# TheRealShamsaba/KnightVision

Measured on AMD Instinct MI355X. Metric: MCTS simulations/sec + self-play games/hour, higher is better.
Workload: dtype fp32

## Files before the change

### include/kv.h

```cpp
#ifndef KV_H
#define KV_H

#include <stddef.h>
#include <stdint.h>

#ifdef __cplusplus
extern "C" {
#endif

#define KV_OK 0
#define KV_EINVAL -1
#define KV_ENOMEM -2
#define KV_EHIP -3
#define KV_EOVERFLOW -4

const char* kv_last_error(void);
int kv_version(void);

typedef struct kv_net kv_net;

size_t kv_net_packed_size(void);
int kv_net_create(int device, kv_net** out);
int kv_net_load(kv_net* net, const float* packed, size_t n_floats);
int kv_net_forward(kv_net* net, const float* planes_dev, int B, float* policy_dev, float* value_dev, void* stream);
// ... 183 lines not shown
                       int8_t* states_after, uint8_t* in_check);
int kv_dev_attacks(int device, const int8_t* states, int n, uint64_t* attacked);
int kv_dev_make_move(int device, int8_t* states, const int* index, int n);
int kv_dev_dirichlet(int device, const uint64_t* seeds, int n, double alpha, int k, int draws, double* out,
                     int64_t* attempts, double* tail);
int kv_dev_eval_cache(int device, int entries, const int8_t* boards, const uint16_t* moves, const int* counts,
                      const uint32_t* logits, const uint32_t* values, int n_rows, const int* step_len, int n_steps,
                      int32_t* hit, uint32_t* out_logits, uint32_t* out_values, int64_t* counters);
int kv_host_libm(int op, const double* x, const double* y, int n, double* out);
int kv_dev_py_random(int device, const uint64_t* seeds, int n, int count, double* out);
int kv_dev_wino88i(int device, const double* V, int rows, const double* U, int K, int digits, int seg, double* M,
                   int8_t* v_digits, int* v_exp);
int kv_dev_wino88i32_out(int device, const float* M, int rows, const float* scale, const float* shift,
                         const float* resid, int fused, float* Y, int8_t* v_digits, int* v_exp);
int kv_dev_tower_front(int device, const int8_t* boards, int nb, int rows, const float* wT, const float* scale,
                       const float* shift, int fused, int8_t* v_digits, int* v_exp);
int kv_dev_tower_back(int device, const float* M, int rows, const float* scale, const float* shift,
                      const float* resid, const float* heads, int fused, float* pfeat, float* value);
int kv_dev_wino88r_out(int device, const double* M, int rows, const float* scale, const float* shift,
                       const float* resid, int fused, float* Y, int8_t* v_digits, int* v_exp);
int kv_dev_net_pair(kv_net* a, kv_net* b, int cu_share, int follow);
int kv_dev_i8gemm_bench(int device, int rows, int K, int variant, int iters, float* avg_us, float* M_out);
int kv_dev_gemm_clock(int device, int rows, int digits, double seconds, double* out);
int kv_dev_out_phases(int device, int rows, int resid, int r3, unsigned long long* stamps, float* us);

#define KV_PGN_OUTCOME_NONE (-128)
typedef struct kv_pgn_record {
    char fen[100];
    char san[12];
    int32_t outcome;
    int32_t game;
} kv_pgn_record;
int kv_pgn_extract(const char* text, size_t len, kv_pgn_record* out, size_t cap, size_t* n_out, size_t* consumed,
                   int64_t* n_games);
int kv_fen_codes(const char* fens, size_t stride, int n, int8_t* codes);
int kv_san_move_index(const char* fens, size_t fen_stride, const char* sans, size_t san_stride, int n,
                      int32_t* out);
int kv_chess_perft(const char* fen, int depth, uint64_t* nodes);
int kv_chess_san(const char* fen, const char* san_in, char* san_out, size_t san_cap, char* fen_after, size_t fen_cap);
int kv_chess_fen(const char* fen_in, char* fen_out, size_t cap);

int kv_tr_conv3x3_f16(const void* x_dev, int n, int ci, const void* w_dev, const float* bias_dev, int co,
                      void* y_dev, void* stream);
int kv_tr_conv3x3_add_f16(const void* x_dev, int n, int ci, const void* w_dev, const float* bias_dev, int co,
                          const void* add_dev, void* y_dev, void* stream);
int kv_tr_conv_weights_f16(const float* w_dev, int co, int ci_real, int ci, void* wf_dev, void* wt_dev, void* stream);
// ... 34 lines not shown
```

### knightvision_amd/_lib.py

```python
from __future__ import annotations

import ctypes as C
import os

HERE = os.path.dirname(os.path.abspath(__file__))
LIB_PATH = os.environ.get("KV_LIB_PATH") or os.path.join(HERE, "libkv.so")

_lib = None


class KVError(RuntimeError):
    pass


class Config(C.Structure):
    _fields_ = [("device", C.c_int), ("slots", C.c_int), ("n_games", C.c_int64), ("game_id_base", C.c_int64),
                ("game_id_stride", C.c_int64), ("seed", C.c_uint64), ("seed_mode", C.c_int),
                ("max_moves", C.c_int), ("batch", C.c_int), ("eps", C.c_double), ("alpha", C.c_double),
                ("sims", C.c_int), ("c_puct", C.c_float), ("eval_mode", C.c_int), ("record_cap", C.c_int64),
                ("recycle", C.c_int), ("precision", C.c_int), ("algo", C.c_int), ("tree_edge_cap", C.c_int),
                ("keep_root_visits", C.c_int), ("eval_cache", C.c_int), ("leaves", C.c_int), ("arena", C.c_int), ("sample_plies", C.c_int),
                ("sim_groups", C.c_int), ("reuse_tree", C.c_int)]


# ... 104 lines not shown
        "kv_root_visits_device": ([vp, vp, sz, P(sz), vp], i),
        "kv_root_moves": ([vp, P(C.c_uint16), sz, P(sz)], i),
        "kv_root_moves_device": ([vp, vp, sz, P(sz), vp], i),
        "kv_records_device": ([vp, vp, sz, P(sz), vp], i),
        "kv_sync": ([vp], i),
        "kv_reset_records": ([vp], i),
        "kv_destroy": ([vp], None),
        "kv_search": ([vp, P(C.c_int8), i, P(SearchParams), P(SearchResult)], i),
        "kv_sizeof_search_result": ([], sz),
        "kv_search_advance": ([vp, i, P(C.c_int32), P(C.c_int8)], i),
        "kv_search_continue": ([vp, i, P(SearchParams), P(SearchResult), P(C.c_int32)], i),
        "kv_search_tree_size": ([vp, i, P(C.c_int32), P(C.c_int32)], i),
        "kv_dev_valid_moves": ([i, P(C.c_int8), i, P(C.c_uint16), i, P(i), P(C.c_int8), P(C.c_uint8)], i),
        "kv_dev_make_move": ([i, P(C.c_int8), P(i), i], i),
        "kv_dev_attacks": ([i, P(C.c_int8), i, P(C.c_uint64)], i),
        "kv_dev_dirichlet": ([i, P(C.c_uint64), i, C.c_double, i, i, P(C.c_double), P(i64), P(C.c_double)], i),
        "kv_dev_py_random": ([i, P(C.c_uint64), i, i, P(C.c_double)], i),
        "kv_dev_eval_cache": ([i, i, P(C.c_int8), P(C.c_uint16), P(i), P(C.c_uint32), P(C.c_uint32), i, P(i), i,
                               P(C.c_int32), P(C.c_uint32), P(C.c_uint32), P(i64)], i),
        "kv_host_libm": ([i, P(C.c_double), P(C.c_double), i, P(C.c_double)], i),
        "kv_dev_wino88i": ([i, P(C.c_double), i, P(C.c_double), i, i, i, P(C.c_double), P(C.c_int8), P(i)], i),
        "kv_dev_i8gemm_bench": ([i, i, i, i, i, P(C.c_float), P(C.c_float)], i),
        "kv_dev_gemm_clock": ([i, i, i, C.c_double, P(C.c_double)], i),
        "kv_dev_net_pair": ([vp, vp, i, i], i),
        "kv_dev_out_phases": ([i, i, i, i, P(C.c_uint64), P(C.c_float)], i),
        "kv_dev_wino88i32_out": ([i, P(C.c_float), i, P(C.c_float), P(C.c_float), P(C.c_float), i, P(C.c_float),
                                  P(C.c_int8), P(i)], i),
        "kv_dev_tower_front": ([i, P(C.c_int8), i, i, P(C.c_float), P(C.c_float), P(C.c_float), i, P(C.c_int8),
                                P(i)], i),
        "kv_dev_tower_back": ([i, P(C.c_float), i, P(C.c_float), P(C.c_float), P(C.c_float), P(C.c_float), i,
                               P(C.c_float), P(C.c_float)], i),
        "kv_dev_wino88r_out": ([i, P(C.c_double), i, P(C.c_float), P(C.c_float), P(C.c_float), i, P(C.c_float),
                                P(C.c_int8), P(i)], i),
        "kv_pgn_extract": ([C.c_char_p, sz, P(PgnRecord), sz, P(sz), P(sz), P(i64)], i),
        "kv_fen_codes": ([C.c_char_p, sz, i, P(C.c_int8)], i),
        "kv_san_move_index": ([C.c_char_p, sz, C.c_char_p, sz, i, P(C.c_int32)], i),
        "kv_chess_perft": ([C.c_char_p, i, P(C.c_uint64)], i),
        "kv_chess_san": ([C.c_char_p, C.c_char_p, C.c_char_p, sz, C.c_char_p, sz], i),
        "kv_chess_fen": ([C.c_char_p, C.c_char_p, sz], i),
        "kv_tr_conv3x3_f16": ([vp, i, i, vp, vp, i, vp, vp], i),
        "kv_tr_conv3x3_add_f16": ([vp, i, i, vp, vp, i, vp, vp, vp], i),
        "kv_tr_conv_weights_f16": ([vp, i, i, i, vp, vp, vp], i),
        "kv_tr_wgrad_workspace": ([i, i, i, P(i)], sz),
        "kv_tr_conv3x3_wgrad_f16": ([vp, vp, i, i, i, i, vp, vp, sz, vp], i),
        "kv_tr_bn_workspace": ([i, i], sz),
        "kv_tr_bn_stats_f16": ([vp, i, i, C.c_float, vp, vp, vp, vp, sz, vp], i),
# ... 4 lines not shown
        "kv_tr_head1x1_f16": ([vp, i, vp, vp, vp, vp], i),
        "kv_tr_head1x1_workspace": ([i], sz),
        "kv_tr_head1x1_backward_f16": ([vp, vp, i, vp, vp, vp, vp, vp, sz, vp], i),
        "kv_tr_policy_loss_f16": ([vp, vp, vp, vp, vp, i, vp, vp, vp, vp], i),
        "kv_tr_policy_loss_backward_f16": ([vp, vp, vp, vp, vp, i, vp, vp, vp, vp, vp, vp], i),
    }
    for name, (args, res) in sig.items():
        if not hasattr(L, name):
            continue
        f = getattr(L, name)
        f.argtypes = args
        f.restype = res
    return L


EXPORTED = ["kv_last_error", "kv_version", "kv_net_packed_size", "kv_net_create", "kv_net_load", "kv_net_forward",
            "kv_net_forward_boards", "kv_net_forward_boards_legal", "kv_net_set_timing", "kv_net_last_timing", "kv_net_destroy", "kv_net_set_precision", "kv_net_set_algo",
            "kv_net_calibration", "kv_engine_calibration",
            "kv_create", "kv_sim_groups_for",
            "kv_load_weights", "kv_load_weights_b", "kv_engine_calibration_b", "kv_run", "kv_set_max_moves", "kv_records", "kv_games", "kv_stats_get", "kv_sizeof_config", "kv_sizeof_stats", "kv_root_visits", "kv_root_visits_device", "kv_root_moves", "kv_root_moves_device", "kv_records_device", "kv_sync", "kv_reset_records", "kv_destroy",
            "kv_search", "kv_sizeof_search_result", "kv_search_advance", "kv_search_continue", "kv_search_tree_size",
            "kv_dev_valid_moves", "kv_dev_make_move", "kv_dev_attacks", "kv_dev_dirichlet", "kv_dev_py_random", "kv_host_libm", "kv_dev_eval_cache",
            "kv_dev_wino88i", "kv_dev_wino88i32_out", "kv_dev_wino88r_out", "kv_dev_tower_front", "kv_dev_tower_back", "kv_dev_i8gemm_bench",
            "kv_dev_gemm_clock", "kv_dev_out_phases", "kv_dev_net_pair",
            "kv_pgn_extract", "kv_fen_codes", "kv_san_move_index", "kv_chess_perft", "kv_chess_san", "kv_chess_fen",
            "kv_tr_conv3x3_f16", "kv_tr_conv3x3_add_f16", "kv_tr_conv_weights_f16", "kv_tr_wgrad_workspace", "kv_tr_conv3x3_wgrad_f16",
            "kv_tr_bn_workspace", "kv_tr_bn_stats_f16", "kv_tr_bn_apply_f16", "kv_tr_bn_backward_f16",
            "kv_tr_channel_sum_f16", "kv_tr_planes_to_nhwc", "kv_tr_head1x1_f16", "kv_tr_head1x1_workspace",
            "kv_tr_head1x1_backward_f16", "kv_tr_policy_loss_f16", "kv_tr_policy_loss_backward_f16"]


def lib():
    global _lib
    if _lib is None:
        import torch
        if not os.path.exists(LIB_PATH):
            raise KVError(f"{LIB_PATH} is missing: run `python -c 'import __graft_entry__ as g; g.build()'` "
                          "(the HIP library is required; there is no CPU fallback)")
        L = _declare(C.CDLL(LIB_PATH))
        if hasattr(L, "kv_sizeof_search_result"):
            assert L.kv_sizeof_search_result() == C.sizeof(SearchResult), "kv_search_result: ctypes mirror differs"
        if hasattr(L, "kv_sizeof_config"):
            assert L.kv_sizeof_config() == C.sizeof(Config), "kv_config: ctypes mirror differs"
            assert L.kv_sizeof_stats() == C.sizeof(Stats), "kv_stats: ctypes mirror differs"
        _lib = L
    return _lib

# ... 6 lines not shown
```

### knightvision_amd/csrc/kv_nn.hip

```cpp
#include <hip/hip_runtime.h>
#include <math.h>
#include <stdarg.h>
#include <stdlib.h>
#include <string.h>

#include <algorithm>
#include <chrono>
#include <mutex>
#include <set>
#include <utility>
#include <vector>

#include "kv_common.h"
#include "kv_wino.h"
#include "kv_wino88.h"
#include "kv_wino88d.h"
#include "kv_wino88i.h"
#include "kv_ref64.h"

namespace kv {

static thread_local char g_err[512];

void set_error(const char* fmt, ...) {
// ... 960 lines not shown
    KV_HIP(hipGetLastError());
    return KV_OK;
}

#ifndef KV_I8F32_NB
#define KV_I8F32_NB 3
#endif
template <int K, int TPW, int ND = 4, int LJ = KV_I8F32_LJ, int NB = KV_I8F32_NB>
static int launch_wino88i32_gemm_lagt(const int8_t* V8, const int* ev, const int8_t* U8, const int* eu, float* M,
                                      int rows, int stride, hipStream_t st) {
    using T = kv::Wino88iTile<kv::kI8DigitsF32>;
    constexpr int bytes = NB * T::STAGE;
    auto kern = kv::wino88i32_gemm_lagt_kernel<K, TPW, LJ, false, ND, NB>;
    KV_HIP(lds_opt_in((const void*)kern, bytes));
    const int tiles = kv::W88_XI * (rows / T::WM) * (512 / T::WN);
    KV_REQUIRE(rows % T::WM == 0 && stride % T::WM == 0 && tiles % (8 * TPW) == 0, KV_EINVAL,
               "wino gemm i8 (lagt): rows %d / stride %d vs tile %d", rows, stride, T::WM);
    hipLaunchKernelGGL(kern, dim3(tiles / TPW), dim3(T::THREADS), bytes, st, V8, ev, U8, eu, M, rows, 512, stride,
                       nullptr);
    KV_HIP(hipGetLastError());
    return KV_OK;
}

template <int K, int TPW>
static int launch_wino88i32_gemm_r3k64(const int8_t* V8, const int* ev, const int8_t* U8, const int* eu, float* M,
                                       int rows, int stride, hipStream_t st, int share = 1) {
    constexpr int bytes = 3 * 4 * 128 * 96 + 2 * TPW * 1024;
    auto kern = kv::wino88i32_gemm_r3k64_kernel<K, TPW>;
    if constexpr (K == 512 && TPW == 5) {
        static const int abl = [] {
            const char* e = getenv("KV_R3K64_ABL");
            return e ? atoi(e) : 0;
        }();
        if (abl == 1) kern = kv::wino88i32_gemm_r3k64_kernel<K, TPW, false, 1>;
        if (abl == 2) kern = kv::wino88i32_gemm_r3k64_kernel<K, TPW, false, 2>;
        if (abl == 3) kern = kv::wino88i32_gemm_r3k64_kernel<K, TPW, false, 3>;
        if (abl == 4) kern = kv::wino88i32_gemm_r3k64_kernel<K, TPW, false, 4>;
        if (abl == 7) kern = kv::wino88i32_gemm_r3k64_kernel<K, TPW, false, 7>;
        if (abl == 8) kern = kv::wino88i32_gemm_r3k64_kernel<K, TPW, false, 8>;
    }
    KV_HIP(lds_opt_in((const void*)kern, bytes));
    const int tiles = kv::W88_XI * (rows / 128) * (512 / 128);
    KV_REQUIRE(rows % 128 == 0 && stride % 128 == 0 && tiles % (8 * TPW) == 0, KV_EINVAL,
               "wino gemm i8 (r3k64): rows %d / stride %d vs tile 128", rows, stride);
    int nwg = tiles / TPW;
    const int cus = gemm_cus(share);
    if (r3_one_round() && cus > 0 && cus % 8 == 0 && nwg > cus && nwg % cus == 0) nwg = cus;
    KV_REQUIRE(nwg % 8 == 0 && tiles % (nwg * TPW) == 0, KV_EINVAL, "wino gemm i8 (r3k64): %d tiles, %d workgroups",
               tiles, nwg);
    hipLaunchKernelGGL(kern, dim3(nwg), dim3(512), bytes, st, V8, ev, U8, eu, M, rows, 512, stride, nullptr);
    KV_HIP(hipGetLastError());
    return KV_OK;
}

static int i8f32_tiles_per_wg(int rows, int share = 1) {
    static const bool off = [] {
        const char* e = getenv("KV_I8F32_TPW");
        return e && e[0] == '1';
    }();
    const int cus = gemm_cus(share);
    const int tiles = kv::W88_XI * (rows / 128) * 4;
    if (off || cus <= 0) return 1;
    const int single = (tiles + cus - 1) / cus;
    for (int t = 5; t >= 4; --t) {
        if (tiles % (8 * t)) continue;
        const int wgs = tiles / t;
        if ((wgs + cus - 1) / cus * t <= single) return t;
    }
    return 1;
}
// ... 1021 lines not shown
    } else {
        constexpr int D = kv::kI8DigitsF32;
        rc = K == 256 ? launch_wino88i_slice<256, D>(du.p, 512, 512, kv::W88_XI, u8.p, eu.p, 0)
                      : launch_wino88i_slice<512, D>(du.p, 512, 512, kv::W88_XI, u8.p, eu.p, 0);
        if (!rc)
            rc = K == 256 ? launch_wino88i_slice<256, D>(dv.p, rows, rows, kv::W88_XI, v8.p, ev.p, 0)
                 : seg    ? launch_wino88i_slice<512, D, double, 2>(dv.p, rows, rows, kv::W88_XI, v8.p, ev.p, 0)
                          : launch_wino88i_slice<512, D>(dv.p, rows, rows, kv::W88_XI, v8.p, ev.p, 0);
        if (!rc)
            rc = K == 256 ? i8f32_gemm<256>(v8.p, ev.p, u8.p, eu.p, dmf.p, rows, rows, false, 0)
                          : i8f32_gemm<512>(v8.p, ev.p, u8.p, eu.p, dmf.p, rows, rows, seg != 0, 0);
    }
    if (rc) return rc;
    KV_HIP(hipDeviceSynchronize());
    if (digits == 5 || r8) {
        KV_HIP(hipMemcpy(M, dm.p, nm * sizeof(double), hipMemcpyDeviceToHost));
    } else {
        std::vector<float> mf(nm);
        KV_HIP(hipMemcpy(mf.data(), dmf.p, nm * sizeof(float), hipMemcpyDeviceToHost));
        for (size_t i = 0; i < nm; ++i) M[i] = mf[i];
    }
    if (v_digits) KV_HIP(hipMemcpy(v_digits, v8.p, nv * digits, hipMemcpyDeviceToHost));
    if (v_exp) KV_HIP(hipMemcpy(v_exp, ev.p, (size_t)kv::W88_XI * rows * nseg * sizeof(int), hipMemcpyDeviceToHost));
    return KV_OK;
}

}

template <bool RESID, bool R3>
static void dev_out_rowform(int form, const float* M, int rows, const float* sc, const float* sh, float* y,
                            int8_t* v8, int* ev) {
    const float* rs = RESID ? y : nullptr;
    if (form == 2)
        (void)launch_wino88i32_outp<RESID, true>(M, rows, rows, sc, sh, rs, y, v8, ev, 0, R3);
    else if (form == 0)
        hipLaunchKernelGGL((kv::wino88i32_out_kernel<RESID, true, 512, R3>), dim3(1, rows), dim3(1024), 0, 0, M, rows,
                           sc, sh, rs, y, v8, ev, 0, 0);
    else
        hipLaunchKernelGGL((kv::wino88i32_out2_kernel<RESID, true, R3>), dim3(1, rows), dim3(1024), 0, 0, M, rows, sc,
                           sh, rs, y, v8, ev, 0, 0);
}

extern "C" {

int kv_dev_wino88i32_out(int device, const float* M, int rows, const float* scale, const float* shift,
                         const float* resid, int fused, float* Y, int8_t* v_digits, int* v_exp) {
// ... 317 lines not shown
                return k5 ? launch_wino88i32_gemm<512, 64, 2, 1, 0, true>(v8.p, ev.p, u8.p, eu.p, m.p, rows, rows, true, 0)
                          : launch_wino88i32_gemm<256, 64, 2, 1, 0, true>(v8.p, ev.p, u8.p, eu.p, m.p, rows, rows, true, 0);
            default: KV_REQUIRE(false, KV_EINVAL, "kv_dev_i8gemm_bench: variant %d", variant);
        }
    };
    int rc;
    for (int w = 0; w < 2; ++w)
        if ((rc = run())) return rc;
    kv::DevEvent e0, e1;
    KV_HIP(e0.create());
    KV_HIP(e1.create());
    KV_HIP(hipEventRecord(e0.e, 0));
    for (int it = 0; it < iters; ++it)
        if ((rc = run())) return rc;
    KV_HIP(hipEventRecord(e1.e, 0));
    KV_HIP(hipEventSynchronize(e1.e));
    float ms = 0.f;
    KV_HIP(hipEventElapsedTime(&ms, e0.e, e1.e));
    *avg_us = 1000.f * ms / iters;
    if (M_out) KV_HIP(hipMemcpy(M_out, m.p, nm * sizeof(float), hipMemcpyDeviceToHost));
    return KV_OK;
}

int kv_dev_gemm_clock(int device, int rows, int digits, double seconds, double* out) {
    KV_REQUIRE(rows > 0 && rows % 128 == 0 && rows <= kMaxBoards && (digits == 3 || digits == 4) && seconds > 0 && out,
               KV_EINVAL, "kv_dev_gemm_clock: bad arguments (rows %d: a multiple of 128, at most %d; digits %d: 3 or 4)",
               rows, kMaxBoards, digits);
    const bool r3 = digits == 3;
    KV_HIP(hipSetDevice(device));
    constexpr int K = 512;
    const size_t lv = (size_t)kv::W88_XI * (K / 32) * rows, lu = (size_t)kv::W88_XI * (K / 32) * 512;
    const size_t nm = (size_t)kv::W88_XI * rows * 512;
    kv::DevBuf<int8_t> v8, u8;
    kv::DevBuf<int> ev, eu;
    kv::DevBuf<float> m;
    kv::DevBuf<unsigned long long> stamps;
    KV_HIP(v8.alloc(lv * 128));
    KV_HIP(u8.alloc(lu * 128));
    KV_HIP(ev.alloc((size_t)kv::W88_XI * rows * 2));
    KV_HIP(eu.alloc((size_t)kv::W88_XI * 512));
    KV_HIP(m.alloc(nm));
    hipLaunchKernelGGL(i8_fill_kernel, dim3((unsigned)((lv * 128 + 255) / 256)), dim3(256), 0, 0, v8.p, lv, ev.p,
                       (size_t)kv::W88_XI * rows * 2, 1234u);
    hipLaunchKernelGGL(i8_fill_kernel, dim3((unsigned)((lu * 128 + 255) / 256)), dim3(256), 0, 0, u8.p, lu, eu.p,
                       (size_t)kv::W88_XI * 512, 99u);
    KV_HIP(hipGetLastError());
    int rc;
    for (int w = 0; w < 3; ++w)
        if ((rc = i8f32_gemm<K>(v8.p, ev.p, u8.p, eu.p, m.p, rows, rows, false, 0, r3))) return rc;
    KV_HIP(hipDeviceSynchronize());
    kv::DevEvent e0, e1;
    KV_HIP(e0.create());
    KV_HIP(e1.create());
    int launches = 0;
    const auto t_start = std::chrono::steady_clock::now();
    KV_HIP(hipEventRecord(e0.e, 0));
    while (std::chrono::duration<double>(std::chrono::steady_clock::now() - t_start).count() < seconds) {
        for (int i = 0; i < 50; ++i)
            if ((rc = i8f32_gemm<K>(v8.p, ev.p, u8.p, eu.p, m.p, rows, rows, false, 0, r3))) return rc;
        launches += 50;
        KV_HIP(hipStreamSynchronize(0));
    }
    KV_HIP(hipEventRecord(e1.e, 0));
    KV_HIP(hipEventSynchronize(e1.e));
    float ms = 0.f;
    KV_HIP(hipEventElapsedTime(&ms, e0.e, e1.e));
    using T = kv::Wino88iTile<kv::kI8DigitsF32>;
    const int tpw = i8f32_tiles_per_wg(rows) >= 4 ? i8f32_tiles_per_wg(rows) : 1;
    const int tiles = kv::W88_XI * (rows / T::WM) * (512 / T::WN), nwg = tiles / tpw;
    KV_REQUIRE(tiles % (8 * tpw) == 0, KV_EINVAL, "kv_dev_gemm_clock: %d tiles, %d per workgroup", tiles, tpw);
    KV_HIP(stamps.alloc((size_t)nwg * 4));
    const int bytes = r3 ? 3 * 4 * 128 * 96 + 2 * tpw * 1024 : KV_I8F32_NB * T::STAGE;
    auto kern = r3 ? (tpw == 5   ? kv::wino88i32_gemm_r3k64_kernel<K, 5, true>
                      : tpw == 4 ? kv::wino88i32_gemm_r3k64_kernel<K, 4, true>
                                 : kv::wino88i32_gemm_r3k64_kernel<K, 1, true>)
                   : (tpw == 5   ? kv::wino88i32_gemm_lagt_kernel<K, 5, KV_I8F32_LJ, true, 4, KV_I8F32_NB>
                      : tpw == 4 ? kv::wino88i32_gemm_lagt_kernel<K, 4, KV_I8F32_LJ, true, 4, KV_I8F32_NB>
                                 : kv::wino88i32_gemm_lagt_kernel<K, 1, KV_I8F32_LJ, true, 4, KV_I8F32_NB>);
    KV_HIP(lds_opt_in((const void*)kern, bytes));
    hipLaunchKernelGGL(kern, dim3(nwg), dim3(T::THREADS), bytes, 0, v8.p, ev.p, u8.p, eu.p, m.p, rows, 512, rows,
                       stamps.p);
    KV_HIP(hipGetLastError());
    KV_HIP(hipDeviceSynchronize());
    std::vector<unsigned long long> h((size_t)nwg * 4);
    KV_HIP(hipMemcpy(h.data(), stamps.p, h.size() * sizeof(unsigned long long), hipMemcpyDeviceToHost));
    std::vector<double> mhz;
    mhz.reserve(nwg);
    for (int b = 0; b < nwg; ++b) {
        const double dt = (double)(h[4 * b + 1] - h[4 * b]), dr = (double)(h[4 * b + 3] - h[4 * b + 2]);
        if (dr > 0) mhz.push_back(dt / dr * 100.0);
    }
    KV_REQUIRE(!mhz.empty(), KV_EHIP, "kv_dev_gemm_clock: no stamp pair advanced");
    std::nth_element(mhz.begin(), mhz.begin() + mhz.size() / 2, mhz.end());
    out[0] = mhz[mhz.size() / 2];
    out[1] = 1000.0 * ms / launches;
    out[2] = launches;
    out[3] = tpw;
    return KV_OK;
}

__global__ void out_phase_fill_kernel(float* M, size_t n, float* sc, float* sh) {
    const size_t i = (size_t)blockIdx.x * blockDim.x + threadIdx.x;
    if (i < n) {
        uint32_t z = (uint32_t)(i * 2654435761u) ^ 0x9e3779b9u;
        z ^= z >> 15;
        z *= 0x2c1b3c6du;
        z ^= z >> 12;
        M[i] = ((float)(z & 0xffffff) / 16777216.0f - 0.5f) * 0.6f;
    }
    if (i < 512) {
        sc[i] = 0.5f + (float)(i % 7) * 0.1f;
        sh[i] = -0.01f * (float)(i % 5);
    }
}

int kv_dev_out_phases(int device, int rows, int resid, int r3, unsigned long long* stamps, float* us) {
    KV_REQUIRE(rows > 0 && rows % 128 == 0 && rows <= kMaxBoards && stamps && us, KV_EINVAL,
               "kv_dev_out_phases: bad arguments (rows %d)", rows);
    KV_HIP(hipSetDevice(device));
    const size_t nm = (size_t)kv::W88_XI * rows * 512, ny = (size_t)rows * 64 * 512;
    kv::DevBuf<float> dm, dsc, dsh, dy;
// ... 183 lines not shown
```

### knightvision_amd/csrc/kv_wino88i.h

```cpp
#pragma once
#include <hip/hip_runtime.h>

#include "kv_common.h"
#include "kv_wino88.h"
#include "kv_wino88d.h"

namespace kv {

constexpr int kI8Digits = 5;
constexpr int kI8DigitsF32 = 4;

typedef int i8x16_t __attribute__((ext_vector_type(4)));
typedef int i32x16_t __attribute__((ext_vector_type(16)));

__device__ inline int i8_row_exponent(unsigned m) {
    if (!m) return 0;
    return (int)(m >> 20) - 1022 + ((m & 0xFE000u) == 0xFE000u ? 1 : 0);
}

__device__ inline int i8_row_exponent_f32(unsigned m) {
    if (!m) return 0;
    return (int)(m >> 23) - 126 + ((m & 0x7F0000u) == 0x7F0000u ? 1 : 0);
}

// ... 788 lines not shown
    }
}
#ifndef KV_R3_M_NT
#define KV_R3_M_NT 1
#endif
template <int K, int TPW, bool STAMP = false, int ABL = 0>
__global__ __launch_bounds__(512) void wino88i32_gemm_r3k64_kernel(const int8_t* __restrict__ V8,
                                                                   const int* __restrict__ ev,
                                                                   const int8_t* __restrict__ U8,
                                                                   const int* __restrict__ eu, float* __restrict__ M,
                                                                   int rows, int cout, int stride,
                                                                   unsigned long long* __restrict__ stamps) {
    unsigned long long t0 = 0, r0 = 0;
    if constexpr (STAMP) {
        t0 = __builtin_amdgcn_s_memtime();
        r0 = __builtin_amdgcn_s_memrealtime();
    }
    constexpr int ND = 3, NB = 3, PD = NB - 1, GL = 6;
    constexpr int NT = 2, WM = 128, WN = 128, WC = 2;
    constexpr int NK = K / 32, NU = NK / 2, NSG = TPW * NU;
    constexpr int PLANE = 128 * 96, STAGE = 4 * PLANE;
    static_assert(NK % 2 == 0 && NU > PD && 8 * GL * 1024 == STAGE, "64-k stages, 6 pieces per wave");
    constexpr double kStep = 0.00390625;

    extern __shared__ __attribute__((aligned(16))) i8x16_t lds_i8k64[];
    char* const L0 = (char*)lds_i8k64;

    const int tid = threadIdx.x;
    const int lane = tid & 63, wave = tid >> 6;
    const int wm = wave / WC, wn = wave % WC;
    const int CT = cout / WN, RT = rows / WM;
    const int nwg = (int)gridDim.x, nv = kv::W88_XI * RT * CT, ng = nv / (nwg * TPW), NST = ng * NSG;
    auto coords = [&](int T, int& xi, int& nb, int& rb) {
        const int vb = (int)blockIdx.x + T * nwg;
        const int idx = (vb & 7) * (nv >> 3) + (vb >> 3);
        xi = idx / (CT * RT);
        nb = (idx % CT) * WN;
        rb = ((idx / CT) % RT) * WM;
    };
    int xis[TPW], nbs[TPW], rbs[TPW];

    const int wu = __builtin_amdgcn_readfirstlane(wave);
    const int op = wu >> 2, chunk = (wu >> 1) & 1, pp0 = 6 * (wu & 1);
    const size_t sstep = (op ? (size_t)cout : (size_t)stride) * 96;
    auto tile_base = [&](int xi, int nb, int rb) {
        return (op ? U8 + (((size_t)xi * NK) * cout + (size_t)nb) * 96 : V8 + (((size_t)xi * NK) * stride + (size_t)rb) * 96) +
// ... 7 lines not shown
        goff[g] = (unsigned)(row * 96 + 16 * (slot ^ ((row >> 4) & 1)));
    }
    const int ldst = (op * 2 + chunk) * PLANE + pp0 * 1024;
    auto issue1 = [&](int g, int s, int sg) {
        if constexpr ((ABL & 1) != 0)
            if (sg >= PD) return;
        const int j = s / NU, ku = s - j * NU;
        const int8_t* base = gb[0];
#pragma unroll
        for (int jj = 1; jj <= TPW; ++jj) base = j == jj ? gb[jj] : base;
        const int8_t* const sb = base + (size_t)(2 * ku) * sstep;
#if KV_COPY_SADDR
        const void* src = (const void*)(sb + goff[g]);
#else
        const void* src = (const void*)(sb + (size_t)(int)goff[g]);
#endif
        __builtin_amdgcn_global_load_lds(src,
                                         (__attribute__((address_space(3))) void*)(L0 + (sg % NB) * STAGE + ldst +
                                                                                   g * 1024),
                                         16, 0, 0);
    };

    const int lr = lane & 31, lh = lane >> 5;
    const int arow = wm * 32 + lr;
    int aoff[2][ND], boff[2][NT][ND];
#pragma unroll
    for (int h = 0; h < 2; ++h)
#pragma unroll
        for (int d = 0; d < ND; ++d) {
            aoff[h][d] = h * PLANE + arow * 96 + 16 * ((2 * d + lh) ^ ((arow >> 4) & 1));
#pragma unroll
            for (int nt = 0; nt < NT; ++nt) {
                const int brow = wn * NT * 32 + nt * 32 + lr;
                boff[h][nt][d] = (2 + h) * PLANE + brow * 96 + 16 * ((2 * d + lh) ^ ((brow >> 4) & 1));
            }
        }

    constexpr int NEX = (TPW * 256 + 511) / 512;
    int* const exl = (int*)(L0 + NB * STAGE);
    for (int gi = 0; gi < ng; ++gi) {
#pragma unroll
    for (int j = 0; j < TPW; ++j) {
        coords(gi * TPW + j, xis[j], nbs[j], rbs[j]);
        gb[j] = tile_base(xis[j], nbs[j], rbs[j]);
    }
    {
// ... 15 lines not shown
    if (gi == 0) {
#pragma unroll
        for (int p = 0; p < PD; ++p)
#pragma unroll
            for (int g = 0; g < GL; ++g) issue1(g, p, p);
    }
#pragma unroll
    for (int j = 0; j < TPW; ++j) {
        i32x16_t acc[ND][NT];
#pragma unroll
        for (int l = 0; l < ND; ++l)
#pragma unroll
            for (int nt = 0; nt < NT; ++nt) acc[l][nt] = i32x16_t{};
        i8x16_t pa[2] = {}, pb[2][NT] = {};
        auto h2 = [&]() {
#pragma unroll
            for (int jb = 1; jb < ND; ++jb)
#pragma unroll
                for (int i = 0; i + jb < ND; ++i)
#pragma unroll
                    for (int nt = 0; nt < NT; ++nt)
                        acc[i + jb][nt] = r3mfma<ABL>(pa[i], pb[jb - 1][nt], acc[i + jb][nt]);
        };
        for (int ku = 0; ku < NU; ++ku) {
            const int s = j * NU + ku, sg = gi * NSG + s;
            const int m = NST - 1 - sg < PD - 1 ? NST - 1 - sg : PD - 1;
            if ((gi > 0 || j > 0) && ku < PD) {
                if (m == 0) vm_lgkm_wait<32>();
                else vm_lgkm_wait<GL + 32>();
            } else {
                if (m == 0) vm_lgkm_wait<0>();
                else vm_lgkm_wait<GL>();
            }
            __builtin_amdgcn_s_barrier();
            asm volatile("" ::: "memory");
            const char* buf = L0 + (sg % NB) * STAGE;
            i8x16_t a0[ND], b0[ND][NT], a1[ND], b1[ND][NT];
#pragma unroll
            for (int d = 0; d < ND; ++d) a0[d] = *(const i8x16_t*)(buf + aoff[0][d]);
#pragma unroll
            for (int nt = 0; nt < NT; ++nt) b0[0][nt] = *(const i8x16_t*)(buf + boff[0][nt][0]);
            __builtin_amdgcn_sched_barrier(0);
            if (ku > 0) h2();
            if (sg + PD < NST) {
                issue1(0, s + PD, sg + PD);
                issue1(1, s + PD, sg + PD);
                issue1(2, s + PD, sg + PD);
            }
#pragma unroll
            for (int jb = 0; jb < ND; ++jb) {
                if (jb + 1 < ND) {
#pragma unroll
                    for (int nt = 0; nt < NT; ++nt) b0[jb + 1][nt] = *(const i8x16_t*)(buf + boff[0][nt][jb + 1]);
                } else {
#pragma unroll
                    for (int d = 0; d < ND; ++d) a1[d] = *(const i8x16_t*)(buf + aoff[1][d]);
#pragma unroll
                    for (int nt = 0; nt < NT; ++nt) b1[0][nt] = *(const i8x16_t*)(buf + boff[1][nt][0]);
                }
                __builtin_amdgcn_sched_barrier(0);
#pragma unroll
                for (int i = 0; i + jb < ND; ++i)
#pragma unroll
                    for (int nt = 0; nt < NT; ++nt)
                        acc[i + jb][nt] = r3mfma<ABL>(a0[i], b0[jb][nt], acc[i + jb][nt]);
                if (jb == 0 && sg + PD < NST) {
                    issue1(3, s + PD, sg + PD);
                    issue1(4, s + PD, sg + PD);
                    issue1(5, s + PD, sg + PD);
                }
            }
#pragma unroll
            for (int nt = 0; nt < NT; ++nt) {
                b1[1][nt] = *(const i8x16_t*)(buf + boff[1][nt][1]);
                b1[2][nt] = *(const i8x16_t*)(buf + boff[1][nt][2]);
            }
            __builtin_amdgcn_sched_barrier(0);
#pragma unroll
            for (int i = 0; i < ND; ++i)
#pragma unroll
                for (int nt = 0; nt < NT; ++nt)
                    acc[i][nt] = r3mfma<ABL>(a1[i], b1[0][nt], acc[i][nt]);
            pa[0] = a1[0];
            pa[1] = a1[1];
#pragma unroll
            for (int nt = 0; nt < NT; ++nt) {
                pb[0][nt] = b1[1][nt];
                pb[1][nt] = b1[2][nt];
            }
            if (j == 0 && ku == 1) {
#pragma unroll
                for (int q = 0; q < NEX; ++q)
                    if (tid + q * 512 < TPW * 256) exg[tid + q * 512] = exv[q];
            }
        }
        h2();
        const int xi = xis[j], n_base = nbs[j], r_base = rbs[j];
        const int* evx = exg + j * 256 + wm * 32;
#pragma unroll
        for (int nt = 0; nt < NT; ++nt) {
            const int col = n_base + wn * NT * 32 + nt * 32 + lr;
            const int ec = (ABL & 8) ? -14 : exg[j * 256 + 128 + wn * NT * 32 + nt * 32 + lr] - 14;
#pragma unroll
            for (int r = 0; r < 16; ++r) {
                const int row = (r & 3) + 8 * (r >> 2) + 4 * lh;
                double mm = (double)acc[ND - 1][nt][r];
#pragma unroll
                for (int l = ND - 2; l >= 0; --l) mm = __builtin_fma(mm, kStep, (double)acc[l][nt][r]);
                const float o = (float)ldexp(mm, ((ABL & 8) ? 0 : evx[row]) + ec);
                if constexpr ((ABL & 4) != 0)
                    asm volatile("" ::"v"(o));
                else if constexpr (KV_R3_M_NT)
                    __builtin_nontemporal_store(o, &M[((size_t)xi * stride + r_base + wm * 32 + row) * cout + col]);
                else
                    M[((size_t)xi * stride + r_base + wm * 32 + row) * cout + col] = o;
            }
        }
    }
    }
    if constexpr (STAMP) {
        const unsigned long long t1 = __builtin_amdgcn_s_memtime(), r1 = __builtin_amdgcn_s_memrealtime();
        if (threadIdx.x < 4) {
            const unsigned long long v = threadIdx.x == 0 ? t0 : threadIdx.x == 1 ? t1 : threadIdx.x == 2 ? r0 : r1;
            stamps[(size_t)blockIdx.x * 4 + threadIdx.x] = v;
        }
    }
}

template <int K, int LJ = 3, int S = 5, int RB = 7, bool RL = false>
__global__ __launch_bounds__(512) void wino88i_gemm_lag5_kernel(const int8_t* __restrict__ V8,
                                                                const int* __restrict__ ev,
                                                                const int8_t* __restrict__ U8,
                                                                const int* __restrict__ eu, double* __restrict__ M,
                                                                int rows, int cout, int stride) {
    constexpr int LEV = 5, NBUF = 3;
    using T = Wino88iTile<S>;
    constexpr int NT = T::NT, WM = T::WM, WN = T::WN, GL = T::GL;
    constexpr int NK = K / 32;
    constexpr int NA = S < LEV - LJ ? S : LEV - LJ;
// ... 1062 lines not shown
```

Before: 329,000.

## Overlap r3k64 GEMM epilogue stores with final MFMA stage in multi-tile workgroups

For workgroups that handle several tiles, the last k-stage is reordered so all MFMAs for the first column tile finish first. Its epilogue (digit recombination, ldexp and stores to M) is then interleaved with the remaining MFMAs for the second column tile using scheduling group barriers, and the trailing barrier is dropped. Address arithmetic for the epilogue is precomputed, and the wait count for in-flight stores is made conditional on the ABL variant. New debug entry points expose a standalone r3 GEMM test and a clock variant with an ABL/share option. The risk is more register pressure and scheduling fragility in a hand-tuned kernel.

```diff
diff --git a/include/kv.h b/include/kv.h
--- a/include/kv.h
+++ b/include/kv.h
@@ -229,6 +229,9 @@
 int kv_dev_net_pair(kv_net* a, kv_net* b, int cu_share, int follow);
 int kv_dev_i8gemm_bench(int device, int rows, int K, int variant, int iters, float* avg_us, float* M_out);
 int kv_dev_gemm_clock(int device, int rows, int digits, double seconds, double* out);
+int kv_dev_r3gemm_clock(int device, int rows, int abl, int share, double seconds, double* out);
+int kv_dev_wino88i_r3(int device, const double* V, int rows, const double* U, int K, int tpw, int nwg, int stride,
+                      int row0, double* M, long long* outside);
 int kv_dev_out_phases(int device, int rows, int resid, int r3, unsigned long long* stamps, float* us);
 
 #define KV_PGN_OUTCOME_NONE (-128)
diff --git a/knightvision_amd/_lib.py b/knightvision_amd/_lib.py
--- a/knightvision_amd/_lib.py
+++ b/knightvision_amd/_lib.py
@@ -150,6 +150,8 @@
         "kv_dev_wino88i": ([i, P(C.c_double), i, P(C.c_double), i, i, i, P(C.c_double), P(C.c_int8), P(i)], i),
         "kv_dev_i8gemm_bench": ([i, i, i, i, i, P(C.c_float), P(C.c_float)], i),
         "kv_dev_gemm_clock": ([i, i, i, C.c_double, P(C.c_double)], i),
+        "kv_dev_r3gemm_clock": ([i, i, i, i, C.c_double, P(C.c_double)], i),
+        "kv_dev_wino88i_r3": ([i, P(C.c_double), i, P(C.c_double), i, i, i, i, i, P(C.c_double), P(i64)], i),
         "kv_dev_net_pair": ([vp, vp, i, i], i),
         "kv_dev_out_phases": ([i, i, i, i, P(C.c_uint64), P(C.c_float)], i),
         "kv_dev_wino88i32_out": ([i, P(C.c_float), i, P(C.c_float), P(C.c_float), P(C.c_float), i, P(C.c_float),
@@ -200,7 +202,7 @@
             "kv_search", "kv_sizeof_search_result", "kv_search_advance", "kv_search_continue", "kv_search_tree_size",
             "kv_dev_valid_moves", "kv_dev_make_move", "kv_dev_attacks", "kv_dev_dirichlet", "kv_dev_py_random", "kv_host_libm", "kv_dev_eval_cache",
             "kv_dev_wino88i", "kv_dev_wino88i32_out", "kv_dev_wino88r_out", "kv_dev_tower_front", "kv_dev_tower_back", "kv_dev_i8gemm_bench",
-            "kv_dev_gemm_clock", "kv_dev_out_phases", "kv_dev_net_pair",
+            "kv_dev_gemm_clock", "kv_dev_r3gemm_clock", "kv_dev_wino88i_r3", "kv_dev_out_phases", "kv_dev_net_pair",
             "kv_pgn_extract", "kv_fen_codes", "kv_san_move_index", "kv_chess_perft", "kv_chess_san", "kv_chess_fen",
             "kv_tr_conv3x3_f16", "kv_tr_conv3x3_add_f16", "kv_tr_conv_weights_f16", "kv_tr_wgrad_workspace", "kv_tr_conv3x3_wgrad_f16",
             "kv_tr_bn_workspace", "kv_tr_bn_stats_f16", "kv_tr_bn_apply_f16", "kv_tr_bn_backward_f16",
diff --git a/knightvision_amd/csrc/kv_nn.hip b/knightvision_amd/csrc/kv_nn.hip
--- a/knightvision_amd/csrc/kv_nn.hip
+++ b/knightvision_amd/csrc/kv_nn.hip
@@ -1006,9 +1006,14 @@
     return KV_OK;
 }
 
+static int r3k64_grid(int tiles, int tpw, int share) {
+    const int nwg = tiles / tpw, cus = gemm_cus(share);
+    return r3_one_round() && cus > 0 && cus % 8 == 0 && nwg > cus && nwg % cus == 0 ? cus : nwg;
+}
+
 template <int K, int TPW>
 static int launch_wino88i32_gemm_r3k64(const int8_t* V8, const int* ev, const int8_t* U8, const int* eu, float* M,
-                                       int rows, int stride, hipStream_t st, int share = 1) {
+                                       int rows, int stride, hipStream_t st, int share = 1, int force_nwg = 0) {
     constexpr int bytes = 3 * 4 * 128 * 96 + 2 * TPW * 1024;
     auto kern = kv::wino88i32_gemm_r3k64_kernel<K, TPW>;
     if constexpr (K == 512 && TPW == 5) {
@@ -1027,9 +1032,7 @@
     const int tiles = kv::W88_XI * (rows / 128) * (512 / 128);
     KV_REQUIRE(rows % 128 == 0 && stride % 128 == 0 && tiles % (8 * TPW) == 0, KV_EINVAL,
                "wino gemm i8 (r3k64): rows %d / stride %d vs tile 128", rows, stride);
-    int nwg = tiles / TPW;
-    const int cus = gemm_cus(share);
-    if (r3_one_round() && cus > 0 && cus % 8 == 0 && nwg > cus && nwg % cus == 0) nwg = cus;
+    const int nwg = force_nwg > 0 ? force_nwg : r3k64_grid(tiles, TPW, share);
     KV_REQUIRE(nwg % 8 == 0 && tiles % (nwg * TPW) == 0, KV_EINVAL, "wino gemm i8 (r3k64): %d tiles, %d workgroups",
                tiles, nwg);
     hipLaunchKernelGGL(kern, dim3(nwg), dim3(512), bytes, st, V8, ev, U8, eu, M, rows, 512, stride, nullptr);
@@ -2097,6 +2100,90 @@
     }
     if (v_digits) KV_HIP(hipMemcpy(v_digits, v8.p, nv * digits, hipMemcpyDeviceToHost));
     if (v_exp) KV_HIP(hipMemcpy(v_exp, ev.p, (size_t)kv::W88_XI * rows * nseg * sizeof(int), hipMemcpyDeviceToHost));
+    return KV_OK;
+}
+
+constexpr unsigned kDevMFill = 0x7fc0de01u;
+
+__global__ void dev_m_outside_kernel(const unsigned* __restrict__ M, size_t n, int stride, int row0, int rows,
+                                     unsigned long long* __restrict__ count) {
+    unsigned long long c = 0;
+    for (size_t i = (size_t)blockIdx.x * blockDim.x + threadIdx.x; i < n; i += (size_t)gridDim.x * blockDim.x) {
+        const int row = (int)((i >> 9) % (size_t)stride);
+        if ((row < row0 || row >= row0 + rows) && M[i] != kDevMFill) ++c;
+    }
+    if (c) atomicAdd(count, c);
+}
+
+int kv_dev_wino88i_r3(int device, const double* V, int rows, const double* U, int K, int tpw, int nwg, int stride,
+                      int row0, double* M, long long* outside) {
+    KV_REQUIRE(V && U && M && outside && rows > 0 && rows % 128 == 0 && (K == 256 || K == 512) && stride % 128 == 0 &&
+                   stride <= kMaxBoards && row0 >= 0 && row0 % 128 == 0 && row0 + rows <= stride &&
+                   (tpw == 0 || tpw == 1 || tpw == 4 || tpw == 5) && nwg >= 0 && (tpw || !nwg),
+               KV_EINVAL, "kv_dev_wino88i_r3: bad arguments (rows %d at row %d of %d: multiples of 128, at most %d; "
+               "K %d 256 or 512; tpw %d 0, 1, 4 or 5; %d workgroups only with a tpw)",
+               rows, row0, stride, kMaxBoards, K, tpw, nwg);
+    KV_HIP(hipSetDevice(device));
+    constexpr int X = kv::W88_XI, D = kv::kI8DigitsF32;
+    const size_t nv = (size_t)X * rows * K, nu = (size_t)X * 512 * K;
+    const size_t nms = (size_t)X * stride * 512, line = 96;
+    kv::DevBuf<double> dv, du;
+    kv::DevBuf<float> dm;
+    kv::DevBuf<int8_t> v8c, v8s, u8;
+    kv::DevBuf<int> evc, evs, eu;
+    kv::DevBuf<unsigned long long> cnt;
+    KV_HIP(dv.alloc(nv));
+    KV_HIP(du.alloc(nu));
+    KV_HIP(v8c.alloc(nv * D));
+    KV_HIP(u8.alloc(nu * D));
+    KV_HIP(evc.alloc((size_t)X * rows));
+    KV_HIP(eu.alloc((size_t)X * 512));
+    KV_HIP(v8s.alloc((size_t)X * (K / 32) * stride * line));
+    KV_HIP(evs.alloc((size_t)X * stride));
+    KV_HIP(dm.alloc(nms));
+    KV_HIP(cnt.alloc(1));
+    KV_HIP(hipMemset(v8s.p, 0, (size_t)X * (K / 32) * stride * line));
+    KV_HIP(hipMemset(evs.p, 0, (size_t)X * stride * sizeof(int)));
+    KV_HIP(hipMemset(cnt.p, 0, sizeof(unsigned long long)));
+    KV_HIP(hipMemsetD32((hipDeviceptr_t)dm.p, (int)kDevMFill, nms));
+    KV_HIP(hipMemcpy(dv.p, V, nv * sizeof(double), hipMemcpyHostToDevice));
+    KV_HIP(hipMemcpy(du.p, U, nu * sizeof(double), hipMemcpyHostToDevice));
+    int rc = K == 256 ? launch_wino88i_slice<256, D, double, 1, false, true>(du.p, 512, 512, X, u8.p, eu.p, 0)
+                      : launch_wino88i_slice<512, D, double, 1, false, true>(du.p, 512, 512, X, u8.p, eu.p, 0);
+    if (!rc)
+        rc = K == 256 ? launch_wino88i_slice<256, D, double, 1, false, true>(dv.p, rows, rows, X, v8c.p, evc.p, 0)
+                      : launch_wino88i_slice<512, D, double, 1, false, true>(dv.p, rows, rows, X, v8c.p, evc.p, 0);
+    if (rc) return rc;
+    KV_HIP(hipMemcpy2D(v8s.p + (size_t)row0 * line, (size_t)stride * line, v8c.p, (size_t)rows * line,
+                       (size_t)rows * line, (size_t)X * (K / 32), hipMemcpyDeviceToDevice));
+    KV_HIP(hipMemcpy2D(evs.p + row0, (size_t)stride * sizeof(int), evc.p, (size_t)rows * sizeof(int),
+                       (size_t)rows * sizeof(int), X, hipMemcpyDeviceToDevice));
+    const int8_t* v8 = v8s.p + (size_t)row0 * line;
+    const int* ev = evs.p + row0;
+    float* m = dm.p + (size_t)row0 * 512;
+    auto gemm = [&](auto kc) -> int {
+        constexpr int KK = decltype(kc)::value;
+        switch (tpw) {
+            case 0: return i8f32_gemm<KK>(v8, ev, u8.p, eu.p, m, rows, stride, false, 0, true);
+            case 1: return launch_wino88i32_gemm_r3k64<KK, 1>(v8, ev, u8.p, eu.p, m, rows, stride, 0, 1, nwg);
+            case 4: return launch_wino88i32_gemm_r3k64<KK, 4>(v8, ev, u8.p, eu.p, m, rows, stride, 0, 1, nwg);
+            default: return launch_wino88i32_gemm_r3k64<KK, 5>(v8, ev, u8.p, eu.p, m, rows, stride, 0, 1, nwg);
+        }
+    };
+    rc = K == 256 ? gemm(std::integral_constant<int, 256>{}) : gemm(std::integral_constant<int, 512>{});
+    if (rc) return rc;
+    hipLaunchKernelGGL(dev_m_outside_kernel, dim3(2048), dim3(256), 0, 0, (const unsigned*)dm.p, nms, stride, row0,
+                       rows, cnt.p);
+    KV_HIP(hipGetLastError());
+    KV_HIP(hipDeviceSynchronize());
+    unsigned long long c = 0;
+    KV_HIP(hipMemcpy(&c, cnt.p, sizeof(c), hipMemcpyDeviceToHost));
+    *outside = (long long)c;
+    std::vector<float> mf((size_t)X * rows * 512);
+    for (int x = 0; x < X; ++x)
+        KV_HIP(hipMemcpy(mf.data() + (size_t)x * rows * 512, m + (size_t)x * stride * 512,
+                         (size_t)rows * 512 * sizeof(float), hipMemcpyDeviceToHost));
+    for (size_t i = 0; i < mf.size(); ++i) M[i] = mf[i];
     return KV_OK;
 }
 
@@ -2460,10 +2547,20 @@
     return KV_OK;
 }
 
-int kv_dev_gemm_clock(int device, int rows, int digits, double seconds, double* out) {
-    KV_REQUIRE(rows > 0 && rows % 128 == 0 && rows <= kMaxBoards && (digits == 3 || digits == 4) && seconds > 0 && out,
-               KV_EINVAL, "kv_dev_gemm_clock: bad arguments (rows %d: a multiple of 128, at most %d; digits %d: 3 or 4)",
-               rows, kMaxBoards, digits);
+}
+
+template <int TPW>
+static auto r3k64_dev_kernel(bool stamp, bool abl) {
+    return stamp ? (abl ? kv::wino88i32_gemm_r3k64_kernel<512, TPW, true, 16> : kv::wino88i32_gemm_r3k64_kernel<512, TPW, true>)
+                 : (abl ? kv::wino88i32_gemm_r3k64_kernel<512, TPW, false, 16> : kv::wino88i32_gemm_r3k64_kernel<512, TPW>);
+}
+
+static int gemm_clock(int device, int rows, int digits, int abl, int share, double seconds, double* out) {
+    KV_REQUIRE(rows > 0 && rows % 128 == 0 && rows <= kMaxBoards && (digits == 3 || digits == 4) && seconds > 0 && out &&
+                   (abl == 0 || (abl == 16 && digits == 3)) && (share == 1 || (share == 2 && digits == 3)),
+               KV_EINVAL, "kv_dev_gemm_clock: bad arguments (rows %d: a multiple of 128, at most %d; digits %d: 3 or 4; "
+               "abl %d: 0, or 16 with 3 digits; share %d: 1, or 2 with 3 digits)",
+               rows, kMaxBoards, digits, abl, share);
     const bool r3 = digits == 3;
     KV_HIP(hipSetDevice(device));
     constexpr int K = 512;
@@ -2483,9 +2580,28 @@
     hipLaunchKernelGGL(i8_fill_kernel, dim3((unsigned)((lu * 128 + 255) / 256)), dim3(256), 0, 0, u8.p, lu, eu.p,
                        (size_t)kv::W88_XI * 512, 99u);
     KV_HIP(hipGetLastError());
+    using T = kv::Wino88iTile<kv::kI8DigitsF32>;
+    const int tpw = i8f32_tiles_per_wg(rows, share) >= 4 ? i8f32_tiles_per_wg(rows, share) : 1;
+    const int tiles = kv::W88_XI * (rows / T::WM) * (512 / T::WN);
+    KV_REQUIRE(tiles % (8 * tpw) == 0, KV_EINVAL, "kv_dev_gemm_clock: %d tiles, %d per workgroup", tiles, tpw);
+    const int nwg = r3 ? r3k64_grid(tiles, tpw, tpw >= 4 ? share : 1) : tiles / tpw;
+    const int bytes = r3 ? 3 * 4 * 128 * 96 + 2 * tpw * 1024 : KV_I8F32_NB * T::STAGE;
+    auto r3kern = [&](bool stamp) {
+        return tpw == 5 ? r3k64_dev_kernel<5>(stamp, abl != 0)
+               : tpw == 4 ? r3k64_dev_kernel<4>(stamp, abl != 0)
+                          : r3k64_dev_kernel<1>(stamp, abl != 0);
+    };
+    if (abl) KV_HIP(lds_opt_in((const void*)r3kern(false), bytes));
+    auto launch = [&]() -> int {
+        if (!abl) return i8f32_gemm<K>(v8.p, ev.p, u8.p, eu.p, m.p, rows, rows, false, 0, r3, share);
+        hipLaunchKernelGGL(r3kern(false), dim3(nwg), dim3(512), bytes, 0, v8.p, ev.p, u8.p, eu.p, m.p, rows, 512, rows,
+                           nullptr);
+        KV_HIP(hipGetLastError());
+        return KV_OK;
+    };
     int rc;
     for (int w = 0; w < 3; ++w)
-        if ((rc = i8f32_gemm<K>(v8.p, ev.p, u8.p, eu.p, m.p, rows, rows, false, 0, r3))) return rc;
+        if ((rc = launch())) return rc;
     KV_HIP(hipDeviceSynchronize());
     kv::DevEvent e0, e1;
     KV_HIP(e0.create());
@@ -2495,7 +2611,7 @@
     KV_HIP(hipEventRecord(e0.e, 0));
     while (std::chrono::duration<double>(std::chrono::steady_clock::now() - t_start).count() < seconds) {
         for (int i = 0; i < 50; ++i)
-            if ((rc = i8f32_gemm<K>(v8.p, ev.p, u8.p, eu.p, m.p, rows, rows, false, 0, r3))) return rc;
+            if ((rc = launch())) return rc;
         launches += 50;
         KV_HIP(hipStreamSynchronize(0));
     }
@@ -2503,15 +2619,8 @@
     KV_HIP(hipEventSynchronize(e1.e));
     float ms = 0.f;
     KV_HIP(hipEventElapsedTime(&ms, e0.e, e1.e));
-    using T = kv::Wino88iTile<kv::kI8DigitsF32>;
-    const int tpw = i8f32_tiles_per_wg(rows) >= 4 ? i8f32_tiles_per_wg(rows) : 1;
-    const int tiles = kv::W88_XI * (rows / T::WM) * (512 / T::WN), nwg = tiles / tpw;
-    KV_REQUIRE(tiles % (8 * tpw) == 0, KV_EINVAL, "kv_dev_gemm_clock: %d tiles, %d per workgroup", tiles, tpw);
     KV_HIP(stamps.alloc((size_t)nwg * 4));
-    const int bytes = r3 ? 3 * 4 * 128 * 96 + 2 * tpw * 1024 : KV_I8F32_NB * T::STAGE;
-    auto kern = r3 ? (tpw == 5   ? kv::wino88i32_gemm_r3k64_kernel<K, 5, true>
-                      : tpw == 4 ? kv::wino88i32_gemm_r3k64_kernel<K, 4, true>
-                                 : kv::wino88i32_gemm_r3k64_kernel<K, 1, true>)
+    auto kern = r3 ? r3kern(true)
                    : (tpw == 5   ? kv::wino88i32_gemm_lagt_kernel<K, 5, KV_I8F32_LJ, true, 4, KV_I8F32_NB>
                       : tpw == 4 ? kv::wino88i32_gemm_lagt_kernel<K, 4, KV_I8F32_LJ, true, 4, KV_I8F32_NB>
                                  : kv::wino88i32_gemm_lagt_kernel<K, 1, KV_I8F32_LJ, true, 4, KV_I8F32_NB>);
@@ -2534,7 +2643,21 @@
     out[1] = 1000.0 * ms / launches;
     out[2] = launches;
     out[3] = tpw;
-    return KV_OK;
+    out[4] = nwg;
+    return KV_OK;
+}
+
+extern "C" {
+
+int kv_dev_gemm_clock(int device, int rows, int digits, double seconds, double* out) {
+    double o[5];
+    const int rc = gemm_clock(device, rows, digits, 0, 1, seconds, out ? o : nullptr);
+    if (!rc) memcpy(out, o, 4 * sizeof(double));
+    return rc;
+}
+
+int kv_dev_r3gemm_clock(int device, int rows, int abl, int share, double seconds, double* out) {
+    return gemm_clock(device, rows, 3, abl, share, seconds, out);
 }
 
 __global__ void out_phase_fill_kernel(float* M, size_t n, float* sc, float* sh) {
diff --git a/knightvision_amd/csrc/kv_wino88i.h b/knightvision_amd/csrc/kv_wino88i.h
--- a/knightvision_amd/csrc/kv_wino88i.h
+++ b/knightvision_amd/csrc/kv_wino88i.h
@@ -834,6 +834,8 @@
     constexpr int PLANE = 128 * 96, STAGE = 4 * PLANE;
     static_assert(NK % 2 == 0 && NU > PD && 8 * GL * 1024 == STAGE, "64-k stages, 6 pieces per wave");
     constexpr double kStep = 0.00390625;
+    constexpr bool SPLIT = TPW > 1;
+    constexpr int MST = (ABL & (4 | 16)) ? 0 : 32;
 
     extern __shared__ __attribute__((aligned(16))) i8x16_t lds_i8k64[];
     char* const L0 = (char*)lds_i8k64;
@@ -887,6 +889,7 @@
     };
 
     const int lr = lane & 31, lh = lane >> 5;
+    const unsigned mlo = (unsigned)(4 * lh * cout + lr) * 4u;
     const int arow = wm * 32 + lr;
     int aoff[2][ND], boff[2][NT][ND];
 #pragma unroll
@@ -948,12 +951,33 @@
                     for (int nt = 0; nt < NT; ++nt)
                         acc[i + jb][nt] = r3mfma<ABL>(pa[i], pb[jb - 1][nt], acc[i + jb][nt]);
         };
+        float* const Mt = M + ((size_t)xis[j] * stride + rbs[j] + wu / WC * 32) * cout + nbs[j] + wu % WC * NT * 32;
+        const int* const evx = exg + j * 256 + wm * 32;
+        auto epi = [&](int nt) {
+            const int ec = (ABL & 8) ? -14 : exg[j * 256 + 128 + wn * NT * 32 + nt * 32 + lr] - 14;
+#pragma unroll
+            for (int r = 0; r < 16; ++r) {
+                const int rowu = (r & 3) + 8 * (r >> 2), row = rowu + 4 * lh;
+                double mm = (double)acc[ND - 1][nt][r];
+#pragma unroll
+                for (int l = ND - 2; l >= 0; --l) mm = __builtin_fma(mm, kStep, (double)acc[l][nt][r]);
+                const float o = (float)ldexp(mm, ((ABL & 8) ? 0 : evx[row]) + ec);
+                float* const mp = (float*)((char*)(Mt + (size_t)rowu * cout + nt * 32) + mlo);
+                if constexpr ((ABL & 4) != 0)
+                    asm volatile("" ::"v"(o));
+                else if constexpr (KV_R3_M_NT)
+                    __builtin_nontemporal_store(o, mp);
+                else
+                    *mp = o;
+            }
+        };
         for (int ku = 0; ku < NU; ++ku) {
             const int s = j * NU + ku, sg = gi * NSG + s;
+            const bool last = SPLIT && ku == NU - 1;
             const int m = NST - 1 - sg < PD - 1 ? NST - 1 - sg : PD - 1;
-            if ((gi > 0 || j > 0) && ku < PD) {
-                if (m == 0) vm_lgkm_wait<32>();
-                else vm_lgkm_wait<GL + 32>();
+            if (MST && (gi > 0 || j > 0) && ku < PD) {
+                if (m == 0) vm_lgkm_wait<MST>();
+                else vm_lgkm_wait<GL + MST>();
             } else {
                 if (m == 0) vm_lgkm_wait<0>();
                 else vm_lgkm_wait<GL>();
@@ -988,7 +1012,7 @@
 #pragma unroll
                 for (int i = 0; i + jb < ND; ++i)
 #pragma unroll
-                    for (int nt = 0; nt < NT; ++nt)
+                    for (int nt = 0; nt < (last && jb > 0 ? 1 : NT); ++nt)
                         acc[i + jb][nt] = r3mfma<ABL>(a0[i], b0[jb][nt], acc[i + jb][nt]);
                 if (jb == 0 && sg + PD < NST) {
                     issue1(3, s + PD, sg + PD);
@@ -1002,17 +1026,47 @@
                 b1[2][nt] = *(const i8x16_t*)(buf + boff[1][nt][2]);
             }
             __builtin_amdgcn_sched_barrier(0);
-#pragma unroll
-            for (int i = 0; i < ND; ++i)
-#pragma unroll
-                for (int nt = 0; nt < NT; ++nt)
-                    acc[i][nt] = r3mfma<ABL>(a1[i], b1[0][nt], acc[i][nt]);
-            pa[0] = a1[0];
-            pa[1] = a1[1];
-#pragma unroll
-            for (int nt = 0; nt < NT; ++nt) {
-                pb[0][nt] = b1[1][nt];
-                pb[1][nt] = b1[2][nt];
+            if (last) {
+#pragma unroll
+                for (int i = 0; i < ND; ++i) acc[i][0] = r3mfma<ABL>(a1[i], b1[0][0], acc[i][0]);
+#pragma unroll
+                for (int jb = 1; jb < ND; ++jb)
+#pragma unroll
+                    for (int i = 0; i + jb < ND; ++i) acc[i + jb][0] = r3mfma<ABL>(a1[i], b1[jb][0], acc[i + jb][0]);
+                __builtin_amdgcn_sched_barrier(0);
+#pragma unroll
+                for (int jb = 1; jb < ND; ++jb)
+#pragma unroll
+                    for (int i = 0; i + jb < ND; ++i) acc[i + jb][1] = r3mfma<ABL>(a0[i], b0[jb][1], acc[i + jb][1]);
+#pragma unroll
+                for (int i = 0; i < ND; ++i) acc[i][1] = r3mfma<ABL>(a1[i], b1[0][1], acc[i][1]);
+#pragma unroll
+                for (int jb = 1; jb < ND; ++jb)
+#pragma unroll
+                    for (int i = 0; i + jb < ND; ++i) acc[i + jb][1] = r3mfma<ABL>(a1[i], b1[jb][1], acc[i + jb][1]);
+                if constexpr ((ABL & (2 | 16)) == 0) {
+                    epi(0);
+#pragma unroll
+                    for (int q = 0; q < 9; ++q) {
+                        __builtin_amdgcn_sched_group_barrier(0x008, 1, 0);
+                        __builtin_amdgcn_sched_group_barrier(0x002, 16, 0);
+                        __builtin_amdgcn_sched_group_barrier(0x040, 2, 0);
+                    }
+                }
+                __builtin_amdgcn_sched_barrier(0);
+            } else {
+#pragma unroll
+                for (int i = 0; i < ND; ++i)
+#pragma unroll
+                    for (int nt = 0; nt < NT; ++nt)
+                        acc[i][nt] = r3mfma<ABL>(a1[i], b1[0][nt], acc[i][nt]);
+                pa[0] = a1[0];
+                pa[1] = a1[1];
+#pragma unroll
+                for (int nt = 0; nt < NT; ++nt) {
+                    pb[0][nt] = b1[1][nt];
+                    pb[1][nt] = b1[2][nt];
+                }
             }
             if (j == 0 && ku == 1) {
 #pragma unroll
@@ -1020,27 +1074,15 @@
                     if (tid + q * 512 < TPW * 256) exg[tid + q * 512] = exv[q];
             }
         }
-        h2();
-        const int xi = xis[j], n_base = nbs[j], r_base = rbs[j];
-        const int* evx = exg + j * 256 + wm * 32;
-#pragma unroll
-        for (int nt = 0; nt < NT; ++nt) {
-            const int col = n_base + wn * NT * 32 + nt * 32 + lr;
-            const int ec = (ABL & 8) ? -14 : exg[j * 256 + 128 + wn * NT * 32 + nt * 32 + lr] - 14;
-#pragma unroll
-            for (int r = 0; r < 16; ++r) {
-                const int row = (r & 3) + 8 * (r >> 2) + 4 * lh;
-                double mm = (double)acc[ND - 1][nt][r];
-#pragma unroll
-                for (int l = ND - 2; l >= 0; --l) mm = __builtin_fma(mm, kStep, (double)acc[l][nt][r]);
-                const float o = (float)ldexp(mm, ((ABL & 8) ? 0 : evx[row]) + ec);
-                if constexpr ((ABL & 4) != 0)
-                    asm volatile("" ::"v"(o));
-                else if constexpr (KV_R3_M_NT)
-                    __builtin_nontemporal_store(o, &M[((size_t)xi * stride + r_base + wm * 32 + row) * cout + col]);
-                else
-                    M[((size_t)xi * stride + r_base + wm * 32 + row) * cout + col] = o;
-            }
+        if constexpr (!SPLIT) h2();
+        if constexpr ((ABL & 16) != 0) {
+#pragma unroll
+            for (int l = 0; l < ND; ++l)
+#pragma unroll
+                for (int nt = 0; nt < NT; ++nt) asm volatile("" ::"v"(acc[l][nt]));
+        } else {
+            if constexpr (!SPLIT || (ABL & 2) != 0) epi(0);
+            epi(1);
         }
     }
     }
```

Measured after the change: 334,800, median of 6. 1.8% higher.
